# UCSD-Comp-Imaging/Nerf-Simple

Measured on AMD Instinct MI355X. Metric: ray-samples/sec at 800x800x128, higher is better.
Workload: dtype f16

## Files before the change

nerf-simple_amd/csrc/mlp_bf16_16.hip:

```cpp
#include "composite_device.h"
#include <utility>

using namespace nerf_layout;

#ifdef NERF_HALF
typedef _Float16 elem_t;
#define NERF_MFMA __builtin_amdgcn_mfma_f32_16x16x32_f16
#define NERF_KERNEL nerf_mlp_f16_16_kernel
#define NERF_LAUNCH nerf_amd_launch_mlp_f16_16
#else
typedef __bf16 elem_t;
#define NERF_MFMA __builtin_amdgcn_mfma_f32_16x16x32_bf16
#define NERF_KERNEL nerf_mlp_bf16_16_kernel
#define NERF_LAUNCH nerf_amd_launch_mlp_bf16_16
#endif
typedef elem_t ex8 __attribute__((ext_vector_type(8)));
typedef elem_t ex2 __attribute__((ext_vector_type(2)));

namespace {

constexpr int NCB = 2;
constexpr int WAVES = 16 / NCB;
constexpr int TILE_PTS = WAVES * 16 * NCB;
__host__ __device__ constexpr int tpc(int L) { return L == 0 ? 8 : 4; }

__host__ __device__ constexpr int layer_chunks(int L) { return (b16_mt(L) + tpc(L) - 1) / tpc(L); }
__host__ __device__ constexpr int chunk_first(int L) {
    int c = 0;
    for (int i = 0; i < L; ++i) c += layer_chunks(i);
    return c;
}
constexpr int NUM_CHUNKS = chunk_first(NUM_LAYERS);
__host__ __device__ constexpr int chunk_layer(int cc) {
    int L = 0;
    while (cc >= layer_chunks(L)) { cc -= layer_chunks(L); ++L; }
    return L;
}
__host__ __device__ constexpr int chunk_tiles(int cc) {
    const int L = chunk_layer(cc), C = cc - chunk_first(L);
    const int left = b16_mt(L) - C * tpc(L);
    return left < tpc(L) ? left : tpc(L);
}
__host__ __device__ constexpr int chunk_kib(int cc) { return chunk_tiles(cc) * b16_ks(chunk_layer(cc)); }
__host__ __device__ constexpr int chunk_off_kib(int cc) {
    const int L = chunk_layer(cc), C = cc - chunk_first(L);
    return b16_layer_off_kib(L) + C * tpc(L) * b16_ks(L);
}

constexpr int LDS_WBUF = 40 * 1024;
constexpr int LDS_BIAS = 0;
constexpr int LDS_W0 = 10 * 1024;
constexpr int LDS_POSD = LDS_W0 + 2 * LDS_WBUF;
constexpr int LDS_POSX = LDS_POSD + WAVES * NCB * 1024;
constexpr int LDS_TOTAL = LDS_POSX + WAVES * NCB * 2048;
constexpr int RING_PTS = 1024;
constexpr int LDS_RING_RAW = LDS_TOTAL;
constexpr int LDS_RING_T = LDS_RING_RAW + RING_PTS * 16;
constexpr int LDS_TOTAL_COMP = LDS_RING_T + RING_PTS * 4;
constexpr int COMP_MAX_N = RING_PTS - TILE_PTS;
static_assert(COMP_MAX_N == FUSED_RENDER_MAX_N, "api.hip routes by this limit");
static_assert(B16_BIAS_FLOATS * 4 <= LDS_W0, "bias table");
static_assert(LDS_TOTAL_COMP <= 160 * 1024 && NUM_CHUNKS % 2 == 0, "LDS budget / parity");
static_assert((RING_PTS & (RING_PTS - 1)) == 0 && RING_PTS % TILE_PTS == 0, "ring indexing");

static_assert(ACT_TILE_PTS == TILE_PTS && MASK_TILE_PTS == TILE_PTS, "activation blocks and mask tiles are the kernel's tiles");

typedef __attribute__((address_space(3))) char lds_char;
typedef __attribute__((address_space(3))) void lds_void;
template <class T>
__device__ __forceinline__ T lds_load(unsigned base, int imm) {
    return *reinterpret_cast<const __attribute__((address_space(3))) T*>(
        reinterpret_cast<lds_char*>(0) + base + imm);
}
template <class T>
__device__ __forceinline__ void lds_store(unsigned base, int imm, const T& v) {
    *reinterpret_cast<__attribute__((address_space(3))) T*>(
        reinterpret_cast<lds_char*>(0) + base + imm) = v;
}

struct Ctx {
    __amdgpu_buffer_rsrc_t wrsrc;
    unsigned wave_goff, lane16;
    unsigned b_wread[2];
    unsigned s_wdst[2];
    unsigned b_bias;
    unsigned b_posx, b_posd;
    int wave, lane;
};

struct State {
    ex8 X[NCB][8], Y[NCB][8];
    f32x4 pend[NCB][2];
    float sigma[NCB], rgb[NCB][3];
    bool bad;
    unsigned posd_off[NCB];
    char* acts;
    long long P;
    long long tile;
    int loff[NCB];
    unsigned mb[NCB][2];
    float amax[4];
    long long mask_tile;
    long long p_end;
    unsigned ring_q0;
    struct WFrag* wf;
};
struct WFrag {
    ex8 a[4];
    f32x4 bias0;
};

template <bool RELU>
__device__ __forceinline__ unsigned pack2(float a, float b) {
    const f32x2 v = {a, b};
    const ex2 r = __builtin_convertvector(v, ex2);
    if constexpr (RELU) {
        const s16x2 z = {0, 0};
        return __builtin_bit_cast(unsigned, __builtin_elementwise_max(__builtin_bit_cast(s16x2, r), z));
    } else {
        return __builtin_bit_cast(unsigned, r);
    }
}

template <int CC>
struct Stage {
    static constexpr int NEXT = (CC + 1) % NUM_CHUNKS;
    static constexpr int PIECES = (chunk_kib(NEXT) + WAVES - 1) / WAVES;
    static constexpr int SRC_OFF = chunk_off_kib(NEXT) * 1024;
    static __device__ __forceinline__ void issue_piece(const Ctx& c, int p) {
        __builtin_amdgcn_raw_ptr_buffer_load_lds(
            c.wrsrc,
            reinterpret_cast<lds_void*>(reinterpret_cast<lds_char*>(0) + c.s_wdst[NEXT & 1] + p * (WAVES * 1024)),
            16, c.lane16, c.wave_goff + (SRC_OFF + p * WAVES * 1024), 0, 0);
    }
    static __device__ __forceinline__ void issue(const Ctx& c) {
#pragma unroll
        for (int p = 0; p < PIECES; ++p) issue_piece(c, p);
    }
};

template <int L, int Q, int SAVE = 0>
__device__ __forceinline__ void epilogue_piece(int i, const f32x4 (&acc)[NCB][2], ex8 (&dst)[NCB][8], State& st) {
    constexpr LayerDesc D = layer_desc(L);
    const int cb = i >> 2, j2 = i & 3;
    if constexpr (Q == 0 && L >= 1 && L <= 9) {
        if (j2 == 0) st.bad |= __builtin_amdgcn_classf(acc[cb][0][0], 0x207);
    }
    if constexpr (L == 10) {
        if (j2 == 0) { st.rgb[cb][0] = acc[cb][0][0]; st.rgb[cb][1] = acc[cb][0][1]; st.rgb[cb][2] = acc[cb][0][2]; }
    } else if constexpr (L == 8 && Q == 8) {
        if (j2 == 0) st.sigma[cb] = acc[cb][0][0];
    } else {
        u32x4 w = __builtin_bit_cast(u32x4, dst[cb][Q]);
        w[j2] = pack2<D.relu != 0>(acc[cb][j2 >> 1][2 * (j2 & 1)], acc[cb][j2 >> 1][2 * (j2 & 1) + 1]);
        dst[cb][Q] = __builtin_bit_cast(ex8, w);
        if constexpr (SAVE == 2) {
            constexpr int GS = (L & 1) * 2 + ((Q >> 2) & 1);
            st.amax[GS] = f8_absmax<D.relu == 0>(((Q & 3) == 0 && i == 0) ? 0.f : st.amax[GS], acc[cb][j2 >> 1][2 * (j2 & 1)],
                                                 acc[cb][j2 >> 1][2 * (j2 & 1) + 1]);
            if constexpr ((Q & 3) == 3) {
                if (i == 4 * NCB - 1) {
                    static_assert(NCB == 2, "store_group_f8 takes the two column blocks of a wave");
                    constexpr int Q0 = Q - 3;
                    char* tb = st.acts + (f8_offset_bytes(L, st.P) + st.tile * F8_BLOCK_BYTES);
                    char* sp = st.acts + (f8_scale_offset_bytes(L, st.P) + st.tile * 64);
                    const __amdgpu_buffer_rsrc_t rs = __builtin_amdgcn_make_buffer_rsrc(tb, 0, (int)F8_BLOCK_BYTES, 0x00020000);
                    const __amdgpu_buffer_rsrc_t rss = __builtin_amdgcn_make_buffer_rsrc(sp, 0, 64, 0x00020000);
                    const u32x4 g0[4] = {__builtin_bit_cast(u32x4, dst[0][Q0]), __builtin_bit_cast(u32x4, dst[0][Q0 + 1]),
                                         __builtin_bit_cast(u32x4, dst[0][Q0 + 2]), __builtin_bit_cast(u32x4, dst[0][Q0 + 3])};
                    const u32x4 g1[4] = {__builtin_bit_cast(u32x4, dst[1][Q0]), __builtin_bit_cast(u32x4, dst[1][Q0 + 1]),
                                         __builtin_bit_cast(u32x4, dst[1][Q0 + 2]), w};
                    store_group_f8<2>(rs, st.loff[0], Q0 * 8192, rss, (int)(threadIdx.x & 63), (int)(threadIdx.x >> 6) * 8 + Q0,
                                      g0, g1, st.amax[GS]);
                }
            }
        }
        if constexpr (SAVE) {
            if (SAVE == 1 && j2 == 3) {
                char* tb = st.acts + (act_offset_bytes(L, st.P) + st.tile * ACT_BLOCK_BYTES);
                const __amdgpu_buffer_rsrc_t rs = __builtin_amdgcn_make_buffer_rsrc(tb, 0, (int)ACT_BLOCK_BYTES, 0x00020000);
                store_granule<2>(rs, st.loff[cb], Q * 16384, w);
            }
            if constexpr (D.relu != 0) {
                static_assert(NCB == 2, "mask layout: two column blocks per wave");
                const unsigned wj = w[j2];
                unsigned t;
                asm("v_pk_min_u16 %0, %1, %2" : "=v"(t) : "v"(wj), "s"(0x00010001u));
                const int pos = (Q & 3) * 4 + j2;
                st.mb[cb][Q >> 2] = pos == 0 ? t : ((t << pos) | st.mb[cb][Q >> 2]);
                if (pos == 15) {
                    char* mp = st.acts + (st.mask_tile + ((long long)L * mask_tiles(st.P) * 4 + (cb * 2 + (Q >> 2))) * 2048);
                    *reinterpret_cast<unsigned*>(mp + (unsigned)(threadIdx.x * 4)) = st.mb[cb][Q >> 2];
                }
            }
        }
    }
}

template <int SAVE>
__host__ __device__ constexpr int pair_vmem_ops(int L, int Q) {
    if (!SAVE || L < 0 || L == 10 || (L == 8 && Q == 8)) return 0;
    const int masks = (layer_desc(L).relu != 0 && (Q & 3) == 3) ? NCB : 0;
    return (SAVE == 2 ? ((Q & 3) == 3 ? F8_GROUP + 1 : 0) : NCB) + masks;
}
template <int SAVE>
__host__ __device__ constexpr int pair_mask_ops(int L, int Q) {
    if (!SAVE || L < 0 || L == 10 || (L == 8 && Q == 8)) return 0;
    return (layer_desc(L).relu != 0 && (Q & 3) == 3) ? NCB : 0;
}

template <int SAVE>
__host__ __device__ constexpr int chunk_pair_vmem_ops(int L, int P0, int N) {
    int n = 0;
    for (int j = 0; j < N; ++j) n += pair_vmem_ops<SAVE>(L, P0 + j);
    return n;
}
template <int SAVE>
__host__ __device__ constexpr int vmem_before_barrier(int L, int PL, int PQ, int pair0, int npair_in, int pend_m0, int pend_per,
                                                      int pair_m0, int mt, int m_limit) {
    int n = 0;
    const int last = 4 * NCB - 1;
    if (PL >= 0) {
        const int masks = pair_mask_ops<SAVE>(PL, PQ), data = pair_vmem_ops<SAVE>(PL, PQ) - masks;
        for (int cb = 0; cb < NCB; ++cb) {
            const int own = 4 * cb + 3;
            if (pend_m0 + own / pend_per < m_limit) n += masks / NCB + (SAVE == 2 ? 0 : data / NCB);
        }
        if (SAVE == 2 && pend_m0 + last / pend_per < m_limit) n += data;
    }
    for (int j = 0; j < npair_in; ++j) {
        const int masks = pair_mask_ops<SAVE>(L, pair0 + j), data = pair_vmem_ops<SAVE>(L, pair0 + j) - masks;
        for (int cb = 0; cb < NCB; ++cb) {
            const int own = 4 * cb + 3;
            if (pair_m0 + j * 2 * mt + own < m_limit) n += masks / NCB + (SAVE == 2 ? 0 : data / NCB);
        }
        if (SAVE == 2 && pair_m0 + j * 2 * mt + last < m_limit) n += data;
    }
    return n;
}
template <int L, int P0, int N, int SAVE, int J = 0>
__device__ __forceinline__ void in_chunk_epilogue(int j, int i, const f32x4 (&acc)[NCB][2], ex8 (&dst)[NCB][8], State& st) {
    if constexpr (J < N) {
        if (j == J) epilogue_piece<L, P0 + J, SAVE>(i, acc, dst, st);
        else in_chunk_epilogue<L, P0, N, SAVE, J + 1>(j, i, acc, dst, st);
    }
}

template <int L, int C, int PL, int PQ, int SAVE>
__device__ __forceinline__ void chunk_step(const Ctx& c, State& st, ex8 (&in)[NCB][8], ex8 (&out)[NCB][8]) {
    constexpr LayerDesc D = layer_desc(L);
    constexpr int KS_CHAIN = D.chain_k / 32;
    constexpr int KS_EXTRA = D.extra_slots / 32;
    constexpr int KS = KS_CHAIN + KS_EXTRA;
    constexpr int CC = chunk_first(L) + C;
    constexpr int NT = chunk_tiles(CC);
    constexpr int RT0 = C * tpc(L);
    constexpr int F = NT * KS;
    constexpr int AHEAD = 4;
    constexpr int BIAS_OFF = LDS_BIAS + (b16_bias_off(L) + 16 * RT0) * 4;
    constexpr int XBLK = D.extra_kind == 1 ? 2048 : 1024;
    constexpr int MT = NCB * KS;
    constexpr int PEND_M0 = (L == 10) ? 0 : (NT * MT >= 4 * NCB + 4 ? 2 : 0);
    constexpr int PEND_PER = (L == 10) ? 2 : 1;
    constexpr int PAIR0 = RT0 / 2;
    constexpr int NPAIR_IN = NT >= 4 ? NT / 2 - 1 : 0;
    constexpr int PAIR_M0 = 2 * MT + (MT >= 4 * NCB + 2 ? 2 : 0);
    static_assert(NT < 4 || NT % 2 == 0, "whole pairs per chunk");
    static_assert(PL < 0 || PL == L || (PL == 8 && PQ == 8) || NCB * PQ >= PEND_M0 + 4 * NCB / PEND_PER,
                  "pending pair finished too late");
    const unsigned wb = c.b_wread[CC & 1];
    const unsigned xb = c.b_posx;
    constexpr int NCC = (CC + 1) % NUM_CHUNKS;
    constexpr int NL = chunk_layer(NCC);
    constexpr int NF = chunk_tiles(NCC) * (layer_desc(NL).chain_k / 32 + layer_desc(NL).extra_slots / 32);
    constexpr int NBIAS_OFF = LDS_BIAS + (b16_bias_off(NL) + 16 * (NCC - chunk_first(NL)) * tpc(NL)) * 4;
    const unsigned nwb = c.b_wread[NCC & 1];
    constexpr int TAIL = 3;
    constexpr int FB = F <= TAIL ? F : F - TAIL;
    constexpr int VMEM_N = vmem_before_barrier<SAVE>(L, PL, PQ, PAIR0, NPAIR_IN, PEND_M0, PEND_PER, PAIR_M0, MT, FB * NCB);
    WFrag& wf = *st.wf;
    auto barrier_and_prefetch = [&]() {
        asm volatile("s_waitcnt lgkmcnt(0)" ::: "memory");
        chunk_barrier<VMEM_N>();
#pragma unroll
        for (int f = 0; f < AHEAD && f < NF; ++f) wf.a[f] = lds_load<ex8>(nwb, f * 1024);
        wf.bias0 = lds_load<f32x4>(c.b_bias, NBIAS_OFF);
        __builtin_amdgcn_sched_barrier(0);
    };

    constexpr int SPREAD = 4;
    constexpr bool DMA_SPREAD = !SAVE && 1 + SPREAD * (Stage<CC>::PIECES - 1) + 8 <= FB * NCB;
    if constexpr (!DMA_SPREAD) Stage<CC>::issue(c);
    __builtin_amdgcn_sched_barrier(0);

    ex8 a[AHEAD];
#pragma unroll
    for (int f = 0; f < AHEAD && f < F; ++f) a[f] = wf.a[f];
    ex8 bx[NCB][KS_EXTRA > 0 ? KS_EXTRA : 1];
    if constexpr (KS_EXTRA > 0) {
#pragma unroll
        for (int cb = 0; cb < NCB; ++cb)
#pragma unroll
            for (int e = 0; e < KS_EXTRA; ++e)
                bx[cb][e] = D.extra_kind == 1 ? lds_load<ex8>(xb, cb * XBLK + e * 1024) : lds_load<ex8>(st.posd_off[cb], e * 1024);
    }
    f32x4 acc[NCB][NT];
    acc[0][0] = wf.bias0;
    for (int cb = 1; cb < NCB; ++cb) acc[cb][0] = acc[0][0];
    __builtin_amdgcn_sched_barrier(0);

    ex8 as_prev = a[0];
    f32x4 c_prev = acc[0][0];
#pragma unroll
    for (int t = 0; t < NT; ++t) {
#pragma unroll
        for (int ks = 0; ks < KS; ++ks) {
            const int f = t * KS + ks;
            if (f == FB) barrier_and_prefetch();
            const ex8 as = a[f % AHEAD];
            if (f + AHEAD < F) a[f % AHEAD] = lds_load<ex8>(wb, (f + AHEAD) * 1024);
            if (t + 1 < NT && ks == KS / 2) {
                acc[0][t + 1 < NT ? t + 1 : 0] = lds_load<f32x4>(c.b_bias, BIAS_OFF + 64 * (t + 1));
                for (int cb = 1; cb < NCB; ++cb) acc[cb][t + 1 < NT ? t + 1 : 0] = acc[0][t + 1 < NT ? t + 1 : 0];
            }
            __builtin_amdgcn_sched_barrier(0);
#pragma unroll
            for (int cb = 0; cb < NCB; ++cb) {
                const int m = f * NCB + cb;
                ex8 bs;
                if (ks < KS_CHAIN) bs = in[cb][ks < KS_CHAIN ? ks : 0];
                else bs = bx[cb][KS_EXTRA > 0 ? (ks - KS_CHAIN < KS_EXTRA ? ks - KS_CHAIN : 0) : 0];
                const f32x4 c_old = acc[cb][t];
                acc[cb][t] = NERF_MFMA(as, bs, c_old, 0, 0, 0);
                asm volatile("" :: "v"(c_prev));
                c_prev = c_old;
                if constexpr (DMA_SPREAD) {
                    if (m % SPREAD == 1 && m / SPREAD < Stage<CC>::PIECES) Stage<CC>::issue_piece(c, m / SPREAD);
                }
                if constexpr (PL >= 0) {
                    if (m >= PEND_M0 && m < PEND_M0 + 4 * NCB / PEND_PER) {
#pragma unroll
                        for (int k = 0; k < PEND_PER; ++k) {
                            const int i = (m - PEND_M0) * PEND_PER + k;
                            if constexpr (PL == L) epilogue_piece<PL, PQ, SAVE>(i, st.pend, out, st);
                            else epilogue_piece<PL, PQ, SAVE>(i, st.pend, in, st);
                        }
                    }
                }
                if constexpr (NPAIR_IN > 0) {
                    const int j = (m - PAIR_M0) / (2 * MT), pm = (m - PAIR_M0) - j * (2 * MT);
                    if (m >= PAIR_M0 && j < NPAIR_IN && pm < 4 * NCB) {
                        f32x4 pr[NCB][2];
                        for (int q_ = 0; q_ < NCB; ++q_) { pr[q_][0] = acc[q_][2 * j]; pr[q_][1] = acc[q_][2 * j + 1]; }
                        in_chunk_epilogue<L, PAIR0, NPAIR_IN, SAVE>(j, pm, pr, out, st);
                    }
                }
                __builtin_amdgcn_sched_barrier(0);
            }
            asm volatile("" :: "v"(as_prev));
            as_prev = as;
            __builtin_amdgcn_sched_barrier(0);
        }
    }
    asm volatile("" :: "v"(as_prev));
    asm volatile("" :: "v"(c_prev));
#pragma unroll
    for (int cb = 0; cb < NCB; ++cb) {
        st.pend[cb][0] = acc[cb][NT >= 2 ? NT - 2 : 0];
        st.pend[cb][1] = acc[cb][NT - 1];
    }
    if constexpr (FB == F) barrier_and_prefetch();
}

__host__ __device__ constexpr int prev_layer(int L, int C) { return C > 0 ? L : L - 1; }
__host__ __device__ constexpr int prev_pair(int L, int C) {
    return C > 0 ? C * tpc(L) / 2 - 1 : (L > 0 ? (L - 1 == 8 ? 8 : b16_mt(L - 1) / 2 - 1) : 0);
}

template <int L, int SAVE, int... Cs>
__device__ __forceinline__ void run_layer_seq(const Ctx& c, State& st, ex8 (&in)[NCB][8], ex8 (&out)[NCB][8],
                                              std::integer_sequence<int, Cs...>) {
    (chunk_step<L, Cs, prev_layer(L, Cs), prev_pair(L, Cs), SAVE>(c, st, in, out), ...);
}
template <int L, int SAVE>
__device__ __forceinline__ void run_layer(const Ctx& c, State& st, ex8 (&in)[NCB][8], ex8 (&out)[NCB][8]) {
    run_layer_seq<L, SAVE>(c, st, in, out, std::make_integer_sequence<int, layer_chunks(L)>{});
}

template <bool RAYS, int SAVE, bool COMP>
__device__ __forceinline__ void stage_inputs(const Ctx& c, const MlpArgs& a, long long tile_base, State& st) {
    const int col = c.lane & 15, g = c.lane >> 4;
    float u_mine = 0.f;
    bool dev_rng = false;
    long long b0 = 0;
    int r0 = 0;
    if constexpr (RAYS) {
        b0 = tile_base / a.N;
        r0 = (int)(tile_base - b0 * a.N);
    }
    const long long p_end = COMP ? st.p_end : a.P;
    const int last_local = (int)(p_end - 1 - tile_base);
    constexpr bool RAY_POSD = RAYS && !SAVE;
    if constexpr (RAY_POSD) {
        const int top = last_local < TILE_PTS - 1 ? last_local : TILE_PTS - 1;
        const int nrays = (int)(split_point(b0, r0, top, a.N).b - b0) + 1;
        for (int idx = threadIdx.x; idx < nrays * 32; idx += WAVES * 64) {
            const int ray = idx >> 5, slot = idx & 31, gg = slot >> 3, sl = slot & 7;
            const float* rp = a.rays + (b0 + ray) * 6 + 3;
            const float dx = rp[0], dy = rp[1], dz = rp[2];
            const float nrm = norm3(dx, dy, dz);
            float val = 0.f;
            if (sl < 6) {
                const int cd = sl >> 1;
                const float dc = __fdiv_rn(cd == 0 ? dx : cd == 1 ? dy : dz, nrm);
                val = enc_lane(to_revolutions(dc), 2 * gg + (sl & 1));
            } else if (sl == 6 && gg < 3) {
                val = __fdiv_rn(gg == 0 ? dx : gg == 1 ? dy : dz, nrm);
            }
            lds_store<elem_t>(LDS_POSD + ray * 64 + slot * 2, 0, (elem_t)val);
        }
    }
    if constexpr (RAYS && NCB == 2) {
        dev_rng = (a.flags & NERF_FLAG_DEVICE_RNG) && !(a.flags & NERF_FLAG_TS_GIVEN);
        if (dev_rng) {
            int lm = c.wave * 32 + (c.lane & 31);
            if (lm > last_local) lm = last_local;
            u_mine = device_rng_uniform(a, split_point(b0, r0, lm, a.N));
        }
    }
#pragma unroll
    for (int cb = 0; cb < NCB; ++cb) {
        long long p = tile_base + c.wave * (16 * NCB) + cb * 16 + col;
        const bool valid = p < p_end;
        st.loff[cb] = valid ? block_lane_offset(g, c.wave * (16 * NCB) + cb * 16 + col) : LOFF_INVALID;
        if constexpr (SAVE == 2) {
            if (cb == 0)
                st.loff[0] = tile_base + c.wave * 32 + 16 * (c.lane >> 5) + col < p_end ? f8_lane_offset(c.lane, c.wave) : LOFF_INVALID;
        }
        if (!valid) p = p_end - 1;
        PointIn pt;
        st.posd_off[cb] = c.b_posd + cb * 1024;
        if constexpr (RAYS) {
            const float u_cb = (NCB == 2) ? __shfl(u_mine, cb * 16 + col) : 0.f;
            int lp = c.wave * (16 * NCB) + cb * 16 + col;
            if (lp > last_local) lp = last_local;
            if (SAVE && a.pts) {
                pt = fetch_point_pts(a, p);
            } else {
                const RaySample rs = split_point(b0, r0, lp, a.N);
                if constexpr (RAY_POSD) st.posd_off[cb] = LDS_POSD + (unsigned)(rs.b - b0) * 64 + g * 16;
                pt = fetch_point_rays<!RAY_POSD>(a, p, rs, u_cb, dev_rng);
                if constexpr (COMP) {
                    if (valid && g == 0)
                        lds_store<float>(((st.ring_q0 + c.wave * (16 * NCB) + cb * 16 + col) & (RING_PTS - 1)) * 4, LDS_RING_T, pt.t);
                }
                if (valid && g == 0 && a.ts_out) a.ts_out[p] = pt.t;
            }
        } else {
            pt = fetch_point_pts(a, p);
        }
        {
            const float xyz[3] = {pt.x, pt.y, pt.z};
            float v[16];
#pragma unroll
            for (int cd = 0; cd < 3; ++cd) {
                const TwoF q = to_revolutions(xyz[cd]);
#pragma unroll
                for (int jj = 0; jj < 5; ++jj) v[cd * 5 + jj] = enc_lane(q, 5 * g + jj);
            }
            v[15] = g == 0 ? pt.x : g == 1 ? pt.y : g == 2 ? pt.z : 0.f;
#pragma unroll
            for (int e = 0; e < 2; ++e) {
                u32x4 r;
#pragma unroll
                for (int i = 0; i < 4; ++i) r[i] = pack2<false>(v[8 * e + 2 * i], v[8 * e + 2 * i + 1]);
                lds_store<u32x4>(c.b_posx, cb * 2048 + e * 1024, r);
            }
        }
        if constexpr (!RAY_POSD) {
            const float dd[3] = {pt.d1, pt.d2, pt.d3};
            float v[8];
#pragma unroll
            for (int cd = 0; cd < 3; ++cd) {
                const TwoF q = to_revolutions(dd[cd]);
#pragma unroll
                for (int jj = 0; jj < 2; ++jj) v[cd * 2 + jj] = enc_lane(q, 2 * g + jj);
            }
            v[6] = g == 0 ? pt.d1 : g == 1 ? pt.d2 : g == 2 ? pt.d3 : 0.f;
            v[7] = 0.f;
            u32x4 r;
#pragma unroll
            for (int i = 0; i < 4; ++i) r[i] = pack2<false>(v[2 * i], v[2 * i + 1]);
            lds_store<u32x4>(c.b_posd, cb * 1024, r);
        }
    }
}

template <bool RAYS, int SAVE, bool COMP>
__device__ __forceinline__ void run_tile(const Ctx& c, const MlpArgs& a, long long tile_base, State& st) {
    stage_inputs<RAYS, SAVE, COMP>(c, a, tile_base, st);
    run_layer<0, SAVE>(c, st, st.X, st.X);
    run_layer<1, SAVE>(c, st, st.X, st.Y);
    run_layer<2, SAVE>(c, st, st.Y, st.X);
    run_layer<3, SAVE>(c, st, st.X, st.Y);
    run_layer<4, SAVE>(c, st, st.Y, st.X);
    run_layer<5, SAVE>(c, st, st.X, st.Y);
    run_layer<6, SAVE>(c, st, st.Y, st.X);
    run_layer<7, SAVE>(c, st, st.X, st.Y);
    run_layer<8, SAVE>(c, st, st.Y, st.X);
    run_layer<9, SAVE>(c, st, st.X, st.Y);
    run_layer<10, SAVE>(c, st, st.Y, st.X);
    epilogue_piece<10, 0>(0, st.pend, st.X, st);
    for (int cb_ = 1; cb_ < NCB; ++cb_) epilogue_piece<10, 0>(4 * cb_, st.pend, st.X, st);
}

__device__ __forceinline__ void flag_nonfinite(const Ctx& c, bool bad) {
    if (bad) __builtin_amdgcn_raw_buffer_store_b32(1u, c.wrsrc, (int)(B16_STATUS_OFF + 4 * NERF_STATUS_WORD_NONFINITE), 0, 0);
}
__device__ __forceinline__ bool finite4(float x, float y, float z, float w) {
    return __builtin_fabsf(x) + __builtin_fabsf(y) + __builtin_fabsf(z) + __builtin_fabsf(w) < __builtin_inff();
}

struct RingSamples {
    unsigned q0;
    __device__ __forceinline__ float t(int i) const {
        return lds_load<float>(((q0 + (unsigned)i) & (RING_PTS - 1)) * 4, LDS_RING_T);
    }
    __device__ __forceinline__ f32x4 c(int i) const {
        return lds_load<f32x4>(((q0 + (unsigned)i) & (RING_PTS - 1)) * 16, LDS_RING_RAW);
    }
};

template <bool RAYS, int SAVE, bool COMP>
__device__ __forceinline__ void kernel_body(const MlpArgs& a, long long ntiles) {
    static_assert(!COMP || (RAYS && !SAVE), "the fused render is the rays-mode inference kernel");
    Ctx c;
    c.wave = __builtin_amdgcn_readfirstlane(threadIdx.x >> 6);
    c.lane = threadIdx.x & 63;
    const char* img = reinterpret_cast<const char*>(a.packed);
    c.wrsrc = __builtin_amdgcn_make_buffer_rsrc(const_cast<char*>(img), 0, (int)B16_IMAGE_BYTES, 0x00020000);
    c.wave_goff = c.wave * 1024;
    c.lane16 = c.lane * 16;
#pragma unroll
    for (int p = 0; p < 2; ++p) {
        c.b_wread[p] = LDS_W0 + p * LDS_WBUF + c.lane * 16;
        c.s_wdst[p] = LDS_W0 + p * LDS_WBUF + c.wave * 1024;
    }
    c.b_bias = (c.lane >> 4) * 16;
    c.b_posx = LDS_POSX + c.wave * (NCB * 2048) + c.lane * 16;
    c.b_posd = LDS_POSD + c.wave * (NCB * 1024) + c.lane * 16;

    {
        const float* bsrc = reinterpret_cast<const float*>(img + (long long)B16_WEIGHT_KIB * 1024);
        for (int i = threadIdx.x; i < B16_BIAS_FLOATS; i += WAVES * 64)
            lds_store<float>(i * 4, LDS_BIAS, bsrc[i]);
        Stage<NUM_CHUNKS - 1>::issue(c);
    }
    asm volatile("s_waitcnt vmcnt(0)" ::: "memory");
    __syncthreads();
    WFrag wf;
    {
        constexpr int F0 = chunk_tiles(0) * (layer_desc(0).chain_k / 32 + layer_desc(0).extra_slots / 32);
#pragma unroll
        for (int f = 0; f < 4 && f < F0; ++f) wf.a[f] = lds_load<ex8>(c.b_wread[0], f * 1024);
        wf.bias0 = lds_load<f32x4>(c.b_bias, LDS_BIAS + b16_bias_off(0) * 4);
    }

    if constexpr (!COMP) {
        for (long long tile = blockIdx.x; tile < ntiles; tile += gridDim.x) {
            const long long tile_base = tile * TILE_PTS;
            asm volatile("" : "+s"(c.wave_goff));
            State st;
            st.wf = &wf;
            st.acts = reinterpret_cast<char*>(a.acts);
            st.P = a.P;
            st.mask_tile = SAVE == 2 ? f8_mask_offset_bytes(0, tile, 0, a.P) : mask_offset_bytes(0, tile, 0, a.P);
            st.tile = tile;
            st.bad = false;
            run_tile<RAYS, SAVE, false>(c, a, tile_base, st);
            bool bad = st.bad;
            if (c.lane < 16) {
#pragma unroll
                for (int cb = 0; cb < NCB; ++cb) {
                    const long long p = tile_base + c.wave * (16 * NCB) + cb * 16 + c.lane;
                    if (p < a.P) {
                        const f32x4 o = {st.rgb[cb][0], st.rgb[cb][1], st.rgb[cb][2], st.sigma[cb]};
                        *reinterpret_cast<f32x4*>(a.raw + p * 4) = o;
                        bad |= !finite4(o[0], o[1], o[2], o[3]);
                    }
                }
            }
            flag_nonfinite(c, bad);
        }
    } else {
        const long long B = a.P / a.N;
        const long long r_lo = (long long)blockIdx.x * B / gridDim.x, r_hi = ((long long)blockIdx.x + 1) * B / gridDim.x;
        const long long range_base = r_lo * a.N;
        const int n_pts = (int)((r_hi - r_lo) * a.N);
        const nerf_composite::RayOut out{a.rgb, a.disp, a.alpha, a.acc, a.w, a.pixels};
        int next_ray = 0, n_complete = 0;
        for (int q_tile = 0; q_tile < n_pts; q_tile += TILE_PTS) {
            const long long tile_base = range_base + q_tile;
            asm volatile("" : "+s"(c.wave_goff));
            State st;
            st.wf = &wf;
            st.acts = nullptr;
            st.P = a.P;
            st.mask_tile = 0;
            st.tile = 0;
            st.p_end = range_base + n_pts;
            st.ring_q0 = (unsigned)q_tile & (RING_PTS - 1);
            st.bad = false;
            run_tile<true, false, true>(c, a, tile_base, st);
            bool bad = st.bad;
            if (c.lane < 16) {
#pragma unroll
                for (int cb = 0; cb < NCB; ++cb) {
                    const int local = c.wave * (16 * NCB) + cb * 16 + c.lane;
                    if (q_tile + local < n_pts) {
                        const f32x4 o = {st.rgb[cb][0], st.rgb[cb][1], st.rgb[cb][2], st.sigma[cb]};
                        lds_store<f32x4>(((st.ring_q0 + local) & (RING_PTS - 1)) * 16, LDS_RING_RAW, o);
                        bad |= !finite4(o[0], o[1], o[2], o[3]);
                    }
                }
            }
            flag_nonfinite(c, bad);
            asm volatile("s_waitcnt lgkmcnt(0)" ::: "memory");
            __builtin_amdgcn_s_barrier();
            asm volatile("" ::: "memory");
            const int done_q = q_tile + TILE_PTS < n_pts ? q_tile + TILE_PTS : n_pts;
            while ((n_complete + 1) * a.N <= done_q) ++n_complete;
            if (n_complete - next_ray >= WAVES || done_q + TILE_PTS - next_ray * a.N > RING_PTS || done_q == n_pts) {
                for (int ray = next_ray + c.wave; ray < n_complete; ray += WAVES) {
                    const long long gray = r_lo + ray;
                    const float* d = a.rays + gray * 6 + 3;
                    const float dnorm = nerf_composite::unit_dir_norm(d[0], d[1], d[2], true);
                    const RingSamples src{(unsigned)(ray * a.N) & (RING_PTS - 1)};
                    nerf_composite::composite_ray(src, a.N, c.lane, dnorm, gray, out);
                }
                next_ray = n_complete;
                asm volatile("s_waitcnt lgkmcnt(0)" ::: "memory");
                __builtin_amdgcn_s_barrier();
                asm volatile("" ::: "memory");
            }
        }
    }
}

template <bool RAYS, bool SAVE, bool COMP>
__global__ __launch_bounds__(WAVES * 64, WAVES / 4) void NERF_KERNEL(MlpArgs a, long long ntiles) {
    extern __shared__ __attribute__((aligned(16))) char smem[];
    (void)smem;
    kernel_body<RAYS, SAVE ? 1 : 0, COMP>(a, ntiles);
}
#ifndef NERF_HALF
__global__ __launch_bounds__(WAVES * 64, WAVES / 4) void nerf_mlp_train_e4m3_kernel(MlpArgs a, long long ntiles) {
    extern __shared__ __attribute__((aligned(16))) char smem[];
    (void)smem;
    kernel_body<true, 2, false>(a, ntiles);
}
#endif

}

extern "C" int NERF_LAUNCH(const MlpArgs* args, int rays_mode, hipStream_t stream) {
    (void)hipGetLastError();
    MlpArgs a = *args;
    if (a.P <= 0) return 0;
    const long long ntiles = (a.P + TILE_PTS - 1) / TILE_PTS;
    const int cus = device_cus();
    const long long grid = ntiles < cus ? ntiles : cus;
    hipError_t e = hipSuccess;
    const bool comp = a.rgb || a.disp || a.acc || a.alpha || a.w || a.pixels;
    if (comp) {
        if (!rays_mode || a.acts || a.N > COMP_MAX_N || a.P / grid + a.N >= (1ll << 31)) return -2;
        auto kern = NERF_KERNEL<true, false, true>;
        e = allow_dynamic_lds(reinterpret_cast<const void*>(kern), LDS_TOTAL_COMP);
        if (e != hipSuccess) return (int)e;
        hipLaunchKernelGGL(kern, dim3((unsigned)grid), dim3(WAVES * 64), LDS_TOTAL_COMP, stream, a, ntiles);
        return (int)hipGetLastError();
    }
#ifdef NERF_HALF
    if (a.acts) return -2;
    auto kern = rays_mode ? NERF_KERNEL<true, false, false> : NERF_KERNEL<false, false, false>;
#else
    if (a.acts && !rays_mode) return -2;
    if ((a.flags & NERF_FLAG_STORE_E4M3) && !a.acts) return -2;
    auto kern = a.acts ? ((a.flags & NERF_FLAG_STORE_E4M3) ? nerf_mlp_train_e4m3_kernel : NERF_KERNEL<true, true, false>)
                       : (rays_mode ? NERF_KERNEL<true, false, false> : NERF_KERNEL<false, false, false>);
#endif
    e = allow_dynamic_lds(reinterpret_cast<const void*>(kern), LDS_TOTAL);
    if (e != hipSuccess) return (int)e;
    hipLaunchKernelGGL(kern, dim3((unsigned)grid), dim3(WAVES * 64), LDS_TOTAL, stream, a, ntiles);
    return (int)hipGetLastError();
}
```

nerf-simple_amd/csrc/nerf_layout.h:

```cpp
#pragma once

#if defined(__HIPCC__)
#define NL_HD __host__ __device__
#else
#define NL_HD
#endif

namespace nerf_layout {

constexpr int NUM_LAYERS = 11;
constexpr int PARAM_COUNT = 595844;
constexpr int FUSED_RENDER_MAX_N = 768;

constexpr int OFF_L0_W = 0;
constexpr int OFF_L0_B = OFF_L0_W + 256 * 63;
constexpr int OFF_L1_W = OFF_L0_B + 256;
constexpr int OFF_SKIP_W = OFF_L1_W + 4 * (256 * 256 + 256);
constexpr int OFF_SKIP_B = OFF_SKIP_W + 256 * 319;
constexpr int OFF_L6_W = OFF_SKIP_B + 256;
constexpr int OFF_SIG_W = OFF_L6_W + 2 * (256 * 256 + 256);
constexpr int OFF_SIG_B = OFF_SIG_W + 256;
constexpr int OFF_L2_W = OFF_SIG_B + 1;
constexpr int OFF_L2_B = OFF_L2_W + 256 * 256;
constexpr int OFF_C0_W = OFF_L2_B + 256;
constexpr int OFF_C0_B = OFF_C0_W + 128 * 283;
constexpr int OFF_C1_W = OFF_C0_B + 128;
constexpr int OFF_C1_B = OFF_C1_W + 3 * 128;
static_assert(OFF_C1_B + 3 == PARAM_COUNT, "parameter offsets");
constexpr int GRAD_BUCKET_SPLIT = OFF_SKIP_W;
static_assert(GRAD_BUCKET_SPLIT % 4 == 0, "16-byte aligned buckets");

struct LayerDesc {
    int w_off, b_off;
    int ld;
    int rows;
    int chain_k;
    int extra_slots;
    int extra_col0;
    int extra_kind;
    int mt;
    int relu;
};

NL_HD constexpr LayerDesc layer_desc(int L) {
    return L == 0 ? LayerDesc{OFF_L0_W, OFF_L0_B, 63, 256, 0, 64, 0, 1, 8, 1}
         : L <= 4 ? LayerDesc{OFF_L1_W + (L - 1) * (256 * 256 + 256),
                              OFF_L1_W + (L - 1) * (256 * 256 + 256) + 256 * 256,
                              256, 256, 256, 0, 0, 0, 8, 1}
         : L == 5 ? LayerDesc{OFF_SKIP_W, OFF_SKIP_B, 319, 256, 256, 64, 256, 1, 8, 1}
         : L <= 7 ? LayerDesc{OFF_L6_W + (L - 6) * (256 * 256 + 256),
                              OFF_L6_W + (L - 6) * (256 * 256 + 256) + 256 * 256,
                              256, 256, 256, 0, 0, 0, 8, 1}
         : L == 8 ? LayerDesc{OFF_L2_W, OFF_L2_B, 256, 256, 256, 0, 0, 0, 9, 0}
         : L == 9 ? LayerDesc{OFF_C0_W, OFF_C0_B, 283, 128, 256, 32, 256, 2, 4, 1}
         :          LayerDesc{OFF_C1_W, OFF_C1_B, 128, 3, 128, 0, 0, 0, 1, 0};
}

NL_HD constexpr int layer_k(int L) { return layer_desc(L).chain_k + layer_desc(L).extra_slots; }

NL_HD constexpr int chain_feat_f32(int s, int g) {
    return 16 * (s >> 2) + 4 * g + (s & 3);
}

NL_HD constexpr int posx_col_f32(int t, int g) {
    return t < 15 ? 3 + 20 * (t / 5) + 5 * g + t % 5
         :          (g < 3 ? g : -1);
}
NL_HD constexpr int posd_col_f32(int t, int g) {
    return t < 6 ? 3 + 8 * (t / 2) + 2 * g + t % 2
         : t == 6 ? (g < 3 ? g : -1)
         :          -1;
}

NL_HD constexpr int src_col_f32(int L, int ks, int g) {
    const LayerDesc d = layer_desc(L);
    const int chain_ks = d.chain_k / 4;
    if (ks < chain_ks) return chain_feat_f32(ks, g);
    const int t = ks - chain_ks;
    const int c = d.extra_kind == 1 ? posx_col_f32(t, g) : posd_col_f32(t, g);
    return c < 0 ? -1 : d.extra_col0 + c;
}

template <class T>
NL_HD inline float weight_at(const T* params, int L, int row, int col) {
    if (col < 0) return 0.f;
    const LayerDesc d = layer_desc(L);
    if (L == 8 && row == 256) return params[OFF_SIG_W + col];
    if (row >= d.rows) return 0.f;
    return params[d.w_off + row * d.ld + col];
}
template <class T>
NL_HD inline float bias_at(const T* params, int L, int row) {
    const LayerDesc d = layer_desc(L);
    if (L == 8 && row == 256) return params[OFF_SIG_B];
    if (row >= d.rows) return 0.f;
    return params[d.b_off + row];
}

NL_HD constexpr int chain_feat_b16(int q, int g, int j) {
    return 32 * q + 16 * (j >> 2) + 4 * g + (j & 3);
}
NL_HD constexpr int src_col_b16(int L, int ks, int g, int j) {
    const LayerDesc d = layer_desc(L);
    const int chain_ks = d.chain_k / 32;
    if (ks < chain_ks) return chain_feat_b16(ks, g, j);
    const int t = 8 * (ks - chain_ks) + j;
    const int c = d.extra_kind == 1 ? posx_col_f32(t, g) : posd_col_f32(t, g);
    return c < 0 ? -1 : d.extra_col0 + c;
}
NL_HD constexpr int b16_mt(int L) { return L == 8 ? 17 : L == 10 ? 1 : layer_desc(L).mt * 2; }
NL_HD constexpr int b16_ks(int L) { return layer_k(L) / 32; }
NL_HD constexpr int b16_layer_off_kib(int L) {
    int o = 0;
    for (int i = 0; i < L; ++i) o += b16_mt(i) * b16_ks(i);
    return o;
}
constexpr int B16_WEIGHT_KIB = b16_layer_off_kib(NUM_LAYERS);
NL_HD constexpr int b16_bias_off(int L) {
    int o = 0;
    for (int i = 0; i < L; ++i) o += b16_mt(i) * 16;
    return o;
}
constexpr int B16_BIAS_FLOATS = b16_bias_off(NUM_LAYERS);
constexpr long long B16_STATUS_OFF = (long long)B16_WEIGHT_KIB * 1024 + B16_BIAS_FLOATS * 4;
constexpr int B16_STATUS_BYTES = 256;
constexpr int NERF_STATUS_WORD_NONFINITE = 0, NERF_STATUS_WORD_WEIGHT_RANGE = 1;
constexpr long long B16_IMAGE_BYTES = B16_STATUS_OFF + B16_STATUS_BYTES;
static_assert(B16_STATUS_OFF % 16 == 0, "aligned status block");

constexpr int NUM_BWD = 10;
struct BwdDesc {
    int wl;
    int rows;
    int chain_k;
    int extra;
    int mask_act;
};
NL_HD constexpr BwdDesc bwd_desc(int b) {
    return b == 0 ? BwdDesc{10, 128, 0, 1, 9}
         : b == 1 ? BwdDesc{9, 256, 128, 0, -1}
         : b == 2 ? BwdDesc{8, 256, 256, 1, 7}
         :          BwdDesc{10 - b, 256, 256, 0, 9 - b};
}
NL_HD constexpr int bwd_ks(int b) { return bwd_desc(b).chain_k / 32 + bwd_desc(b).extra; }
NL_HD constexpr int bwd_mt(int b) { return bwd_desc(b).rows / 16; }
NL_HD constexpr int bwd_src_out(int b, int ks, int g, int j) {
    const BwdDesc d = bwd_desc(b);
    if (ks < d.chain_k / 32) return chain_feat_b16(ks, g, j);
    return b == 0 ? ((g == 0 && j < 3) ? j : -1) : ((g == 0 && j == 0) ? 256 : -1);
}
NL_HD constexpr int bwd_layer_off_kib(int b) {
    int o = 0;
    for (int i = 0; i < b; ++i) o += bwd_mt(i) * bwd_ks(i);
    return o;
}
constexpr int BWD_WEIGHT_KIB = bwd_layer_off_kib(NUM_BWD);
constexpr long long BWD_IMAGE_BYTES = (long long)BWD_WEIGHT_KIB * 1024;

NL_HD constexpr int act_width(int L) { return L == 9 ? 128 : 256; }
constexpr int ACT_TILE_PTS = 256;
constexpr long long ACT_BLOCK_BYTES = 256 * 512;
NL_HD constexpr long long act_tiles(long long P) { return (P + ACT_TILE_PTS - 1) / ACT_TILE_PTS; }
NL_HD constexpr long long act_layer_stride(long long P) { return act_tiles(P) * ACT_BLOCK_BYTES; }
NL_HD constexpr long long act_offset_bytes(int L, long long P) { return (long long)L * act_layer_stride(P); }
NL_HD constexpr long long act_elem_offset(int L, long long p, int f, long long P) {
    return act_offset_bytes(L, P) + (p / ACT_TILE_PTS) * ACT_BLOCK_BYTES
         + ((long long)(f / 8) * ACT_TILE_PTS + p % ACT_TILE_PTS) * 16 + (f % 8) * 2;
}
NL_HD constexpr long long acts_bf16_bytes(long long P) { return 10 * act_layer_stride(P); }

constexpr int MASK_TILE_PTS = 256;
NL_HD constexpr long long mask_tiles(long long P) { return (P + MASK_TILE_PTS - 1) / MASK_TILE_PTS; }
NL_HD constexpr long long mask_region_offset(long long P) { return acts_bf16_bytes(P); }
NL_HD constexpr long long mask_offset_bytes(int L, long long tile, int dword, long long P) {
    return mask_region_offset(P) + (((long long)L * mask_tiles(P) + tile) * 4 + dword) * 2048;
}
NL_HD constexpr long long acts_total_bytes(long long P) { return acts_bf16_bytes(P) + 10 * mask_tiles(P) * 8192; }

constexpr long long F8_BLOCK_BYTES = 256 * 256;
constexpr int F8_SCALE_BYTES_PER_BLOCK = 8;
NL_HD constexpr long long f8_layer_stride(long long P) { return act_tiles(P) * F8_BLOCK_BYTES; }
NL_HD constexpr long long f8_offset_bytes(int L, long long P) { return (long long)L * f8_layer_stride(P); }
NL_HD constexpr long long f8_elem_offset(int L, long long p, int f, long long P) {
    return f8_offset_bytes(L, P) + (p / ACT_TILE_PTS) * F8_BLOCK_BYTES + ((long long)(f / 16) * ACT_TILE_PTS + p % ACT_TILE_PTS) * 16 + f % 16;
}
NL_HD constexpr long long f8_scale_layer_stride(long long P) { return act_tiles(P) * (ACT_TILE_PTS / 32) * F8_SCALE_BYTES_PER_BLOCK; }
NL_HD constexpr long long f8_scale_offset_bytes(int L, long long P) { return 10 * f8_layer_stride(P) + (long long)L * f8_scale_layer_stride(P); }
NL_HD constexpr long long f8_data_bytes(long long P) { return 10 * f8_layer_stride(P) + 10 * f8_scale_layer_stride(P); }
NL_HD constexpr long long f8_mask_region_offset(long long P) { return (f8_data_bytes(P) + 255) / 256 * 256; }
NL_HD constexpr long long f8_mask_offset_bytes(int L, long long tile, int dword, long long P) {
    return f8_mask_region_offset(P) + (((long long)L * mask_tiles(P) + tile) * 4 + dword) * 2048;
}
NL_HD constexpr long long f8_acts_total_bytes(long long P) { return f8_mask_region_offset(P) + 10 * mask_tiles(P) * 8192; }
NL_HD constexpr long long f8_narrow_block_bytes(int W) { return (long long)(W / 16) * ACT_TILE_PTS * 16; }
NL_HD constexpr long long f8_narrow_scale_offset(int W, long long P) { return act_tiles(P) * f8_narrow_block_bytes(W); }
NL_HD constexpr long long f8_narrow_bytes(int W, long long P) { return f8_narrow_scale_offset(W, P) + f8_scale_layer_stride(P); }

NL_HD constexpr int f32_mt(int L) { return L == 8 ? 17 : L == 10 ? 1 : layer_desc(L).mt * 2; }
NL_HD constexpr int f32_ks(int L) { return layer_k(L) / 4; }
NL_HD constexpr int f32_chunk_kib(int L) { return (layer_k(L) / 16 + 3) / 4 * 4; }
NL_HD constexpr int f32_layer_off_kib(int L) {
    int o = 0;
    for (int i = 0; i < L; ++i) o += f32_mt(i) * f32_chunk_kib(i);
    return o;
}
constexpr int F32_WEIGHT_KIB = f32_layer_off_kib(NUM_LAYERS);
NL_HD constexpr int f32_bias_off(int L) {
    int o = 0;
    for (int i = 0; i < L; ++i) o += f32_mt(i) * 16;
    return o;
}
constexpr int F32_BIAS_FLOATS = f32_bias_off(NUM_LAYERS);
constexpr long long F32_PACKED_BYTES = (long long)F32_WEIGHT_KIB * 1024 + F32_BIAS_FLOATS * 4;
NL_HD constexpr int f32_num_chunks() {
    int c = 0;
    for (int i = 0; i < NUM_LAYERS; ++i) c += f32_mt(i);
    return c;
}
constexpr int F32_NUM_CHUNKS = f32_num_chunks();

}
```

nerf-simple_amd/csrc/pack.hip:

```cpp
#include "nerf_device.h"

using namespace nerf_layout;

namespace {

template <class T>
__global__ void pack_b16_kernel(const float* __restrict__ params, T* __restrict__ out, unsigned* __restrict__ status) {
    const long long total = (long long)B16_WEIGHT_KIB * 512;
    for (long long e = blockIdx.x * (long long)blockDim.x + threadIdx.x; e < total;
         e += (long long)gridDim.x * blockDim.x) {
        const int kib = (int)(e >> 9);
        int L = 0;
        while (L + 1 < NUM_LAYERS && kib >= b16_layer_off_kib(L + 1)) ++L;
        const int rel = kib - b16_layer_off_kib(L);
        const int rt = rel / b16_ks(L), s = rel % b16_ks(L);
        const int lane = (int)(e >> 3) & 63, j = (int)e & 7;
        const int row = 16 * rt + (lane & 15), g = lane >> 4;
        const float wv = weight_at(params, L, row, src_col_b16(L, s, g, j));
        const T cv = (T)wv;
        out[e] = cv;
        if (!(__builtin_fabsf((float)cv) < __builtin_inff())) status[NERF_STATUS_WORD_WEIGHT_RANGE] = 1u;
    }
}

__global__ void pack_bwd_kernel(const float* __restrict__ params, __bf16* __restrict__ out) {
    const long long total = (long long)BWD_WEIGHT_KIB * 512;
    for (long long e = blockIdx.x * (long long)blockDim.x + threadIdx.x; e < total;
         e += (long long)gridDim.x * blockDim.x) {
        const int kib = (int)(e >> 9);
        int b = 0;
        while (b + 1 < NUM_BWD && kib >= bwd_layer_off_kib(b + 1)) ++b;
        const int rel = kib - bwd_layer_off_kib(b);
        const int rt = rel / bwd_ks(b), s = rel % bwd_ks(b);
        const int lane = (int)(e >> 3) & 63, j = (int)e & 7;
        const int in_col = 16 * rt + (lane & 15), g = lane >> 4;
        const int o = bwd_src_out(b, s, g, j);
        out[e] = (__bf16)(o < 0 ? 0.f : weight_at(params, bwd_desc(b).wl, o, in_col));
    }
}

__global__ void pack_f32_kernel(const float* __restrict__ params, float* __restrict__ out) {
    const long long total = (long long)F32_WEIGHT_KIB * 256;
    for (long long e = blockIdx.x * (long long)blockDim.x + threadIdx.x; e < total;
         e += (long long)gridDim.x * blockDim.x) {
        const int kib = (int)(e >> 8);
        int L = 0;
        while (L + 1 < NUM_LAYERS && kib >= f32_layer_off_kib(L + 1)) ++L;
        const int rel = kib - f32_layer_off_kib(L);
        const int ck = f32_chunk_kib(L);
        const int t = rel / ck, q = rel % ck;
        const int lane = (int)(e >> 2) & 63, i = (int)e & 3;
        const int ks = 4 * q + i;
        float v = 0.f;
        if (ks < f32_ks(L)) {
            const int row = 16 * t + (lane & 15), g = lane >> 4;
            v = weight_at(params, L, row, src_col_f32(L, ks, g));
        }
        out[e] = v;
    }
}

__global__ void pack_bias_kernel(const float* __restrict__ params, float* __restrict__ out, unsigned* __restrict__ status) {
    static_assert(B16_BIAS_FLOATS == F32_BIAS_FLOATS, "one bias table layout");
    if (status && blockIdx.x == 0 && threadIdx.x < B16_STATUS_BYTES / 4) status[threadIdx.x] = 0u;
    for (int e = blockIdx.x * blockDim.x + threadIdx.x; e < F32_BIAS_FLOATS; e += gridDim.x * blockDim.x) {
        int L = 0;
        while (L + 1 < NUM_LAYERS && e >= f32_bias_off(L + 1)) ++L;
        out[e] = bias_at(params, L, e - f32_bias_off(L));
    }
}

__global__ void pack_clear_status_kernel(unsigned* __restrict__ status) {
    if (threadIdx.x < B16_STATUS_BYTES / 4) status[threadIdx.x] = 0u;
}
constexpr int PACK_TRAIN_BIAS_FRAGS = (F32_BIAS_FLOATS + 511) / 512;
constexpr int PACK_TRAIN_FRAGS = B16_WEIGHT_KIB + BWD_WEIGHT_KIB + PACK_TRAIN_BIAS_FRAGS;
__global__ __launch_bounds__(256) void pack_train_kernel(const float* __restrict__ params, __bf16* __restrict__ img,
                                                         float* __restrict__ bias, __bf16* __restrict__ bwd,
                                                         unsigned* __restrict__ status) {
    bool bad = false;
    const int frag = blockIdx.x;
    if (frag < B16_WEIGHT_KIB) {
        const int kib = frag;
        int L = 0;
        while (L + 1 < NUM_LAYERS && kib >= b16_layer_off_kib(L + 1)) ++L;
        const int rel = kib - b16_layer_off_kib(L);
        const int rt = rel / b16_ks(L), s_ = rel % b16_ks(L);
#pragma unroll
        for (int h = 0; h < 2; ++h) {
            const int e = threadIdx.x + 256 * h;
            const int lane = e >> 3, j = e & 7;
            const __bf16 cv = (__bf16)weight_at(params, L, 16 * rt + (lane & 15), src_col_b16(L, s_, lane >> 4, j));
            img[(long long)kib * 512 + e] = cv;
            bad |= !(__builtin_fabsf((float)cv) < __builtin_inff());
        }
    } else if (frag < B16_WEIGHT_KIB + BWD_WEIGHT_KIB) {
        const int kib = frag - B16_WEIGHT_KIB;
        int b = 0;
        while (b + 1 < NUM_BWD && kib >= bwd_layer_off_kib(b + 1)) ++b;
        const int rel = kib - bwd_layer_off_kib(b);
        const int rt = rel / bwd_ks(b), s_ = rel % bwd_ks(b);
        const int wl = bwd_desc(b).wl;
#pragma unroll
        for (int h = 0; h < 2; ++h) {
            const int e = threadIdx.x + 256 * h;
            const int lane = e >> 3, j = e & 7;
            const int o = bwd_src_out(b, s_, lane >> 4, j);
            bwd[(long long)kib * 512 + e] = (__bf16)(o < 0 ? 0.f : weight_at(params, wl, o, 16 * rt + (lane & 15)));
        }
    } else {
#pragma unroll
        for (int h = 0; h < 2; ++h) {
            const int q = (frag - B16_WEIGHT_KIB - BWD_WEIGHT_KIB) * 512 + threadIdx.x + 256 * h;
            if (q < F32_BIAS_FLOATS) {
                int L = 0;
                while (L + 1 < NUM_LAYERS && q >= f32_bias_off(L + 1)) ++L;
                bias[q] = bias_at(params, L, q - f32_bias_off(L));
            }
        }
    }
    if (bad) status[NERF_STATUS_WORD_WEIGHT_RANGE] = 1u;
}

}

extern "C" int nerf_amd_launch_pack_train(const float* params, void* packed_bf16, void* packed_bwd, hipStream_t stream) {
    (void)hipGetLastError();
    char* img = reinterpret_cast<char*>(packed_bf16);
    unsigned* status = reinterpret_cast<unsigned*>(img + B16_STATUS_OFF);
    hipLaunchKernelGGL(pack_clear_status_kernel, dim3(1), dim3(64), 0, stream, status);
    hipLaunchKernelGGL(pack_train_kernel, dim3(PACK_TRAIN_FRAGS), dim3(256), 0, stream, params, reinterpret_cast<__bf16*>(img),
                       reinterpret_cast<float*>(img + (long long)B16_WEIGHT_KIB * 1024), reinterpret_cast<__bf16*>(packed_bwd), status);
    return (int)hipGetLastError();
}

extern "C" int nerf_amd_launch_pack(const float* params, void* packed, int precision, hipStream_t stream) {
    (void)hipGetLastError();
    char* img = reinterpret_cast<char*>(packed);
    if (precision == 1 || precision == 2) {
        unsigned* status = reinterpret_cast<unsigned*>(img + B16_STATUS_OFF);
        hipLaunchKernelGGL(pack_bias_kernel, dim3(10), dim3(256), 0, stream, params,
                           reinterpret_cast<float*>(img + (long long)B16_WEIGHT_KIB * 1024), status);
        if (precision == 1)
            hipLaunchKernelGGL(pack_b16_kernel<__bf16>, dim3(1024), dim3(256), 0, stream, params,
                               reinterpret_cast<__bf16*>(img), status);
        else
            hipLaunchKernelGGL(pack_b16_kernel<_Float16>, dim3(1024), dim3(256), 0, stream, params,
                               reinterpret_cast<_Float16*>(img), status);
    } else if (precision == 3) {
        hipLaunchKernelGGL(pack_bwd_kernel, dim3(1024), dim3(256), 0, stream, params,
                           reinterpret_cast<__bf16*>(img));
    } else {
        hipLaunchKernelGGL(pack_f32_kernel, dim3(1024), dim3(256), 0, stream, params,
                           reinterpret_cast<float*>(img));
        hipLaunchKernelGGL(pack_bias_kernel, dim3(10), dim3(256), 0, stream, params,
                           reinterpret_cast<float*>(img + (long long)F32_WEIGHT_KIB * 1024), static_cast<unsigned*>(nullptr));
    }
    return (int)hipGetLastError();
}
```

Baseline: 1.208 billion.

## Fold feature linear layer into color layer weights for the f16 path

For the half-precision path, the linear feature layer (layer 8 without activation) is algebraically merged into the next color layer. The packer precomputes the product of the two weight matrices and folds the bias, so the kernel runs only the sigma tile of layer 8 and skips 256x256 MACs per point. The chunk count drops from 38 to 34 and the ping-pong buffers are adjusted. The risk is different rounding, since the product is formed in fp32 and then rounded to f16.

```diff
diff --git a/nerf-simple_amd/csrc/mlp_bf16_16.hip b/nerf-simple_amd/csrc/mlp_bf16_16.hip
--- a/nerf-simple_amd/csrc/mlp_bf16_16.hip
+++ b/nerf-simple_amd/csrc/mlp_bf16_16.hip
@@ -24,7 +24,16 @@
 constexpr int TILE_PTS = WAVES * 16 * NCB;
 __host__ __device__ constexpr int tpc(int L) { return L == 0 ? 8 : 4; }
 
-__host__ __device__ constexpr int layer_chunks(int L) { return (b16_mt(L) + tpc(L) - 1) / tpc(L); }
+#ifdef NERF_HALF
+constexpr bool FOLD = true;
+#else
+constexpr bool FOLD = false;
+#endif
+__host__ __device__ constexpr int k_mt(int L) { return FOLD ? fold_mt(L) : b16_mt(L); }
+__host__ __device__ constexpr int k_layer_off_kib(int L) { return FOLD ? fold_layer_off_kib(L) : b16_layer_off_kib(L); }
+__host__ __device__ constexpr int k_bias_off(int L) { return FOLD ? fold_bias_off(L) : b16_bias_off(L); }
+
+__host__ __device__ constexpr int layer_chunks(int L) { return (k_mt(L) + tpc(L) - 1) / tpc(L); }
 __host__ __device__ constexpr int chunk_first(int L) {
     int c = 0;
     for (int i = 0; i < L; ++i) c += layer_chunks(i);
@@ -38,13 +47,13 @@
 }
 __host__ __device__ constexpr int chunk_tiles(int cc) {
     const int L = chunk_layer(cc), C = cc - chunk_first(L);
-    const int left = b16_mt(L) - C * tpc(L);
+    const int left = k_mt(L) - C * tpc(L);
     return left < tpc(L) ? left : tpc(L);
 }
 __host__ __device__ constexpr int chunk_kib(int cc) { return chunk_tiles(cc) * b16_ks(chunk_layer(cc)); }
 __host__ __device__ constexpr int chunk_off_kib(int cc) {
     const int L = chunk_layer(cc), C = cc - chunk_first(L);
-    return b16_layer_off_kib(L) + C * tpc(L) * b16_ks(L);
+    return k_layer_off_kib(L) + C * tpc(L) * b16_ks(L);
 }
 
 constexpr int LDS_WBUF = 40 * 1024;
@@ -61,6 +70,7 @@
 static_assert(COMP_MAX_N == FUSED_RENDER_MAX_N, "api.hip routes by this limit");
 static_assert(B16_BIAS_FLOATS * 4 <= LDS_W0, "bias table");
 static_assert(LDS_TOTAL_COMP <= 160 * 1024 && NUM_CHUNKS % 2 == 0, "LDS budget / parity");
+static_assert(NUM_CHUNKS == (FOLD ? 34 : 38), "chunks per tile");
 static_assert((RING_PTS & (RING_PTS - 1)) == 0 && RING_PTS % TILE_PTS == 0, "ring indexing");
 
 static_assert(ACT_TILE_PTS == TILE_PTS && MASK_TILE_PTS == TILE_PTS, "activation blocks and mask tiles are the kernel's tiles");
@@ -257,7 +267,7 @@
     constexpr int RT0 = C * tpc(L);
     constexpr int F = NT * KS;
     constexpr int AHEAD = 4;
-    constexpr int BIAS_OFF = LDS_BIAS + (b16_bias_off(L) + 16 * RT0) * 4;
+    constexpr int BIAS_OFF = LDS_BIAS + (k_bias_off(L) + 16 * RT0) * 4;
     constexpr int XBLK = D.extra_kind == 1 ? 2048 : 1024;
     constexpr int MT = NCB * KS;
     constexpr int PEND_M0 = (L == 10) ? 0 : (NT * MT >= 4 * NCB + 4 ? 2 : 0);
@@ -273,7 +283,7 @@
     constexpr int NCC = (CC + 1) % NUM_CHUNKS;
     constexpr int NL = chunk_layer(NCC);
     constexpr int NF = chunk_tiles(NCC) * (layer_desc(NL).chain_k / 32 + layer_desc(NL).extra_slots / 32);
-    constexpr int NBIAS_OFF = LDS_BIAS + (b16_bias_off(NL) + 16 * (NCC - chunk_first(NL)) * tpc(NL)) * 4;
+    constexpr int NBIAS_OFF = LDS_BIAS + (k_bias_off(NL) + 16 * (NCC - chunk_first(NL)) * tpc(NL)) * 4;
     const unsigned nwb = c.b_wread[NCC & 1];
     constexpr int TAIL = 3;
     constexpr int FB = F <= TAIL ? F : F - TAIL;
@@ -374,7 +384,7 @@
 
 __host__ __device__ constexpr int prev_layer(int L, int C) { return C > 0 ? L : L - 1; }
 __host__ __device__ constexpr int prev_pair(int L, int C) {
-    return C > 0 ? C * tpc(L) / 2 - 1 : (L > 0 ? (L - 1 == 8 ? 8 : b16_mt(L - 1) / 2 - 1) : 0);
+    return C > 0 ? C * tpc(L) / 2 - 1 : (L > 0 ? (L - 1 == 8 ? 8 : k_mt(L - 1) / 2 - 1) : 0);
 }
 
 template <int L, int SAVE, int... Cs>
@@ -507,9 +517,11 @@
     run_layer<5, SAVE>(c, st, st.X, st.Y);
     run_layer<6, SAVE>(c, st, st.Y, st.X);
     run_layer<7, SAVE>(c, st, st.X, st.Y);
+    ex8 (&c_in)[NCB][8] = FOLD ? st.Y : st.X;
+    ex8 (&c_out)[NCB][8] = FOLD ? st.X : st.Y;
     run_layer<8, SAVE>(c, st, st.Y, st.X);
-    run_layer<9, SAVE>(c, st, st.X, st.Y);
-    run_layer<10, SAVE>(c, st, st.Y, st.X);
+    run_layer<9, SAVE>(c, st, c_in, c_out);
+    run_layer<10, SAVE>(c, st, c_out, c_in);
     epilogue_piece<10, 0>(0, st.pend, st.X, st);
     for (int cb_ = 1; cb_ < NCB; ++cb_) epilogue_piece<10, 0>(4 * cb_, st.pend, st.X, st);
 }
@@ -563,7 +575,7 @@
         constexpr int F0 = chunk_tiles(0) * (layer_desc(0).chain_k / 32 + layer_desc(0).extra_slots / 32);
 #pragma unroll
         for (int f = 0; f < 4 && f < F0; ++f) wf.a[f] = lds_load<ex8>(c.b_wread[0], f * 1024);
-        wf.bias0 = lds_load<f32x4>(c.b_bias, LDS_BIAS + b16_bias_off(0) * 4);
+        wf.bias0 = lds_load<f32x4>(c.b_bias, LDS_BIAS + k_bias_off(0) * 4);
     }
 
     if constexpr (!COMP) {
diff --git a/nerf-simple_amd/csrc/nerf_layout.h b/nerf-simple_amd/csrc/nerf_layout.h
--- a/nerf-simple_amd/csrc/nerf_layout.h
+++ b/nerf-simple_amd/csrc/nerf_layout.h
@@ -128,6 +128,30 @@
 constexpr long long B16_IMAGE_BYTES = B16_STATUS_OFF + B16_STATUS_BYTES;
 static_assert(B16_STATUS_OFF % 16 == 0, "aligned status block");
 
+constexpr int FOLD_SIGMA_TILE = 16;
+NL_HD constexpr int fold_rt0(int L) { return L == 8 ? FOLD_SIGMA_TILE : 0; }
+NL_HD constexpr int fold_mt(int L) { return L == 8 ? 1 : b16_mt(L); }
+NL_HD constexpr int fold_layer_off_kib(int L) { return b16_layer_off_kib(L) + fold_rt0(L) * b16_ks(L); }
+NL_HD constexpr int fold_bias_off(int L) { return b16_bias_off(L) + fold_rt0(L) * 16; }
+NL_HD constexpr int b16_padded_macs(bool fold) {
+    int m = 0;
+    for (int L = 0; L < NUM_LAYERS; ++L) m += (fold ? fold_mt(L) : b16_mt(L)) * 16 * layer_k(L);
+    return m;
+}
+static_assert(b16_padded_macs(false) == 600064 && b16_padded_macs(true) == 600064 - 65536, "padded MACs per point");
+template <class T>
+NL_HD inline float fold_weight_at(const T* params, int row, int col) {
+    float s = 0.f;
+    for (int k = 0; k < 256; ++k) s = __builtin_fmaf(params[OFF_C0_W + row * 283 + k], params[OFF_L2_W + k * 256 + col], s);
+    return s;
+}
+template <class T>
+NL_HD inline float fold_bias_at(const T* params, int row) {
+    float s = 0.f;
+    for (int k = 0; k < 256; ++k) s = __builtin_fmaf(params[OFF_C0_W + row * 283 + k], params[OFF_L2_B + k], s);
+    return params[OFF_C0_B + row] + s;
+}
+
 constexpr int NUM_BWD = 10;
 struct BwdDesc {
     int wl;
diff --git a/nerf-simple_amd/csrc/pack.hip b/nerf-simple_amd/csrc/pack.hip
--- a/nerf-simple_amd/csrc/pack.hip
+++ b/nerf-simple_amd/csrc/pack.hip
@@ -4,7 +4,7 @@
 
 namespace {
 
-template <class T>
+template <class T, bool FOLD>
 __global__ void pack_b16_kernel(const float* __restrict__ params, T* __restrict__ out, unsigned* __restrict__ status) {
     const long long total = (long long)B16_WEIGHT_KIB * 512;
     for (long long e = blockIdx.x * (long long)blockDim.x + threadIdx.x; e < total;
@@ -16,7 +16,9 @@
         const int rt = rel / b16_ks(L), s = rel % b16_ks(L);
         const int lane = (int)(e >> 3) & 63, j = (int)e & 7;
         const int row = 16 * rt + (lane & 15), g = lane >> 4;
-        const float wv = weight_at(params, L, row, src_col_b16(L, s, g, j));
+        const int col = src_col_b16(L, s, g, j);
+        const float wv = (FOLD && L == 9 && s < layer_desc(9).chain_k / 32) ? fold_weight_at(params, row, col)
+                                                                            : weight_at(params, L, row, col);
         const T cv = (T)wv;
         out[e] = cv;
         if (!(__builtin_fabsf((float)cv) < __builtin_inff())) status[NERF_STATUS_WORD_WEIGHT_RANGE] = 1u;
@@ -60,13 +62,14 @@
     }
 }
 
-__global__ void pack_bias_kernel(const float* __restrict__ params, float* __restrict__ out, unsigned* __restrict__ status) {
+__global__ void pack_bias_kernel(const float* __restrict__ params, float* __restrict__ out, unsigned* __restrict__ status, int fold) {
     static_assert(B16_BIAS_FLOATS == F32_BIAS_FLOATS, "one bias table layout");
     if (status && blockIdx.x == 0 && threadIdx.x < B16_STATUS_BYTES / 4) status[threadIdx.x] = 0u;
     for (int e = blockIdx.x * blockDim.x + threadIdx.x; e < F32_BIAS_FLOATS; e += gridDim.x * blockDim.x) {
         int L = 0;
         while (L + 1 < NUM_LAYERS && e >= f32_bias_off(L + 1)) ++L;
-        out[e] = bias_at(params, L, e - f32_bias_off(L));
+        const int row = e - f32_bias_off(L);
+        out[e] = (fold && L == 9 && row < layer_desc(9).rows) ? fold_bias_at(params, row) : bias_at(params, L, row);
     }
 }
 
@@ -140,12 +143,12 @@
     if (precision == 1 || precision == 2) {
         unsigned* status = reinterpret_cast<unsigned*>(img + B16_STATUS_OFF);
         hipLaunchKernelGGL(pack_bias_kernel, dim3(10), dim3(256), 0, stream, params,
-                           reinterpret_cast<float*>(img + (long long)B16_WEIGHT_KIB * 1024), status);
+                           reinterpret_cast<float*>(img + (long long)B16_WEIGHT_KIB * 1024), status, precision == 2 ? 1 : 0);
         if (precision == 1)
-            hipLaunchKernelGGL(pack_b16_kernel<__bf16>, dim3(1024), dim3(256), 0, stream, params,
+            hipLaunchKernelGGL((pack_b16_kernel<__bf16, false>), dim3(1024), dim3(256), 0, stream, params,
                                reinterpret_cast<__bf16*>(img), status);
         else
-            hipLaunchKernelGGL(pack_b16_kernel<_Float16>, dim3(1024), dim3(256), 0, stream, params,
+            hipLaunchKernelGGL((pack_b16_kernel<_Float16, true>), dim3(1024), dim3(256), 0, stream, params,
                                reinterpret_cast<_Float16*>(img), status);
     } else if (precision == 3) {
         hipLaunchKernelGGL(pack_bwd_kernel, dim3(1024), dim3(256), 0, stream, params,
@@ -154,7 +157,7 @@
         hipLaunchKernelGGL(pack_f32_kernel, dim3(1024), dim3(256), 0, stream, params,
                            reinterpret_cast<float*>(img));
         hipLaunchKernelGGL(pack_bias_kernel, dim3(10), dim3(256), 0, stream, params,
-                           reinterpret_cast<float*>(img + (long long)F32_WEIGHT_KIB * 1024), static_cast<unsigned*>(nullptr));
+                           reinterpret_cast<float*>(img + (long long)F32_WEIGHT_KIB * 1024), static_cast<unsigned*>(nullptr), 0);
     }
     return (int)hipGetLastError();
 }
```

Result: faster. 1.347 billion (median of 6 runs) (+11.5%).
